# td-kwj-zp2023/webgpu-msm-twisted-edwards

Hardware: AMD Instinct MI355X
Metric: MSMs/sec at n=2^20 Twisted-Edwards BLS12 (pipelined throughput = 1000/ms_per_step; single-MSM latency in latency_ms) (higher is better)
Workload: dtype u32

## Files before the change

### webgpu-msm-twisted-edwards_amd/csrc/kernels.hip.hpp

```cpp
#pragma once
#include <hip/hip_runtime.h>
#include "curve.hpp"

namespace te {

#define TE_BATCH_MAX 8
struct batch_ptrs { const uint4* p[TE_BATCH_MAX]; };
struct batch_slabs { uint32_t s[TE_BATCH_MAX]; };

struct digits_params {
  uint32_t half[10];
  uint32_t zero_digit;
  uint32_t sc_stride;
  uint32_t n, nst;
  int num_windows;
  int w_first, w_step, nw_local;
  uint32_t half_code, logS, P, CH, chunk_len;
};

struct pnt_slot { uint4 q[8]; };
__device__ __forceinline__ void prep_points_block(uint32_t blk, uint4* __restrict__ lds, const uint4* __restrict__ pts, pnt_slot* __restrict__ recs, uint32_t n) {
  const uint32_t t = threadIdx.x, base = blk * 256u;
  const bool active = t < 256u;
  const uint32_t pieces_in = (n - base < 256u ? n - base : 256u) * 4u;
// ... 355 lines not shown
    prep_points_block(blk, lds4, in.p[row], recs + (size_t)row_slab.s[row] * n, n);
  }
}


struct piece_regs { uint4 k[5], ia[5], ib[5]; };
template <bool PK>
__device__ __forceinline__ void load_piece(const uint16_t* __restrict__ keys_row, const uint32_t* __restrict__ idx_row, uint32_t a, uint32_t b,
                                           uint32_t t, bool with_idx, piece_regs& r, uint32_t& head, uint32_t& total) {
  const uint32_t a_al = a & ~7u;
  head = a - a_al; total = head + (b - a);
  const uint32_t groups = (total + 7u) >> 3;
  const uint4* k4 = reinterpret_cast<const uint4*>(keys_row + a_al);
  const uint4* i4 = reinterpret_cast<const uint4*>(idx_row + a_al);
#pragma unroll
  for (int c = 0; c < 5; c++) {
    const uint32_t gi = min((uint32_t)c * 256u + t, groups - 1u);
    if (!PK) r.k[c] = k4[gi];
    if (PK || with_idx) { r.ia[c] = i4[2 * gi]; r.ib[c] = i4[2 * gi + 1]; }
  }
}
template <bool PK> __device__ __forceinline__ void piece_group(const piece_regs& r, int c, uint32_t (&kv)[8], uint32_t (&iv)[8]) {
  const uint32_t w[8] = {r.ia[c].x, r.ia[c].y, r.ia[c].z, r.ia[c].w, r.ib[c].x, r.ib[c].y, r.ib[c].z, r.ib[c].w};
  if (PK) {
#pragma unroll
    for (int e = 0; e < 8; e++) { kv[e] = ((w[e] >> 23) & 0xffu) | ((w[e] >> 31) << 15); iv[e] = w[e] & 0x7fffffu; }
  } else {
    unpack8(r.k[c], kv);
#pragma unroll
    for (int e = 0; e < 8; e++) iv[e] = w[e];
  }
}
static_assert(5u * 256u * 8u >= TE_L2_CAP + 8u, "five groups per thread hold a piece");

__device__ __forceinline__ bool l2_piece_of_block(uint32_t bx, const uint32_t* __restrict__ pc, uint32_t P, uint32_t overflow_pieces, uint32_t* sm, uint32_t* pj, uint32_t& p, uint32_t& j) {
  if (bx < P) { p = bx; j = 0u; return true; }
  const uint32_t t = threadIdx.x, x = bx - P;
  if (x >= overflow_pieces) return false;
  const uint32_t c = t < P ? pc[t] : 0u;
  const uint32_t ov = c ? (c + TE_L2_CAP - 1u) / TE_L2_CAP - 1u : 0u;
  uint32_t tot;
  const uint32_t ex = block_excl_scan(ov, sm, tot);
  if (x >= tot) return false;
  if (x >= ex && x < ex + ov) { pj[0] = t; pj[1] = x - ex + 1u; }
  __syncthreads();
  p = pj[0]; j = pj[1];
  __syncthreads();
  return true;
}

#define TE_COMBINE_SMALL 16u
#define TE_GIANT_RUN 256u
#define TE_SEG_INVALID 0xffffffffu
#define TE_HIST_COPIES 32u
struct plan_args {
  const uint32_t* part_start; const uint32_t* part_count; const uint32_t* seg_part_base;
  uint32_t *bucket_start, *bucket_cursor, *seg_base, *seg_bucket, *seg_lenv, *size_hist, *split_list;
  uint32_t* split_count;
  uint32_t* chunk_list;
  uint32_t seg_len, cap_w, chunk_cap;
};
struct plan_lds { uint32_t h[1024]; uint32_t sm[17]; uint32_t giant[256 * 3]; uint32_t n_giant; };
__device__ __forceinline__ uint32_t seg_plan_block(uint32_t p, uint32_t k, uint32_t cnt_in, const sort_geom& sg, const plan_args& a, plan_lds& L,
                                                   uint32_t pstart, uint32_t pcount, uint32_t sbase) {
  const uint32_t t = threadIdx.x, P = sg.P, S = sg.S, B = sg.B, seg_len = a.seg_len;
  uint32_t* const h = L.h; uint32_t* const sm = L.sm; uint32_t* const giant = L.giant;
  __syncthreads();
  for (uint32_t j = t; j < 1024u; j += 256u) h[j] = 0u;
  if (t == 0) L.n_giant = 0u;
  const bool mine = t < S;
  const uint32_t g = k * B + p * S + (mine ? t : 0u);
  const uint32_t cnt = mine ? cnt_in : 0u;
  const uint32_t nparts = mine ? max(1u, (cnt + seg_len - 1u) / seg_len) : 0u;
  uint32_t bt, bt2;
  const uint32_t ex = block_excl_scan(cnt, sm, bt);
  const uint32_t ex2 = block_excl_scan(nparts, sm, bt2);
  const uint32_t bs = pstart + ex, sb = sbase + ex2;
  if (mine) {
    a.bucket_start[g] = bs; a.bucket_cursor[g] = bs; a.seg_base[g] = sb;
    if (nparts <= TE_COMBINE_SMALL) {
      for (uint32_t part = 0; part < nparts; part++) {
        const uint32_t len = cnt > part * seg_len ? min(seg_len, cnt - part * seg_len) : 0u;
        a.seg_bucket[sb + part] = g; a.seg_lenv[sb + part] = len;
        atomicAdd(&h[min(len, 1023u)], 1u);
      }
      if (nparts > 1u) a.split_list[atomicAdd(&a.split_count[0], 1u)] = g;
    } else {
      const uint32_t j = atomicAdd(&L.n_giant, 1u);
      giant[3 * j] = g; giant[3 * j + 1] = sb; giant[3 * j + 2] = cnt;
      atomicAdd(&a.split_count[1], 1u);
    }
  }
  {
    const uint32_t first = sbase, used = bt2;
    const uint32_t cap = p + 1u == P ? (k + 1u) * a.cap_w - first : S + pcount / seg_len;
    for (uint32_t j = used + t; j < cap; j += 256u) { a.seg_bucket[first + j] = TE_SEG_INVALID; a.seg_lenv[first + j] = TE_SEG_INVALID; }
  }
  __syncthreads();
  const uint32_t ng = L.n_giant;
  for (uint32_t j = 0; j < ng; j++) {
    const uint32_t gg = giant[3 * j], sb0 = giant[3 * j + 1], c0 = giant[3 * j + 2];
    const uint32_t np = (c0 + seg_len - 1u) / seg_len;
    for (uint32_t part = t; part < np; part += 256u) {
      const uint32_t len = min(seg_len, c0 - part * seg_len);
      a.seg_bucket[sb0 + part] = gg; a.seg_lenv[sb0 + part] = len;
      atomicAdd(&h[min(len, 1023u)], 1u);
      if ((part & (TE_GIANT_RUN - 1u)) == 0) { const uint32_t ci = atomicAdd(&a.split_count[2], 1u); if (ci < a.chunk_cap) { a.chunk_list[2 * ci] = gg; a.chunk_list[2 * ci + 1] = part; } }
    }
  }
  __syncthreads();
  uint32_t* my_hist = a.size_hist + ((k * P + p) % TE_HIST_COPIES) * 1024u;
  for (uint32_t j = t; j < 1024u; j += 256u) if (h[j]) atomicAdd(&my_hist[j], h[j]);
  __syncthreads();
  return ex;
}

struct l2_args {
  const uint16_t* part_keys; const uint32_t* part_idx; const uint32_t* part_start; const uint32_t* part_count;
  uint32_t* bucket_count; uint32_t* sorted;
  uint32_t* part_ticket;
  sort_geom g; plan_args pa;
};
#define TE_L2A_LDS_WORDS (3u * 256u + 32u + TE_L2_LIST)
static_assert(sizeof(plan_lds) <= TE_L2_LIST * 4u, "the plan's LDS fits into the list area");
template <bool PK>
__global__ void __launch_bounds__(256, TE_L2_WAVES) k_l2_local(l2_args a) {
  __shared__ uint32_t lds[TE_L2A_LDS_WORDS];
  uint32_t* const cnt_s = lds; uint32_t* const off_s = lds + 256; uint32_t* const sm = lds + 768; uint32_t* const pj = lds + 768 + 17;
  uint32_t* const list = lds + 768 + 32;
  plan_lds& PL = *reinterpret_cast<plan_lds*>(list);
  const sort_geom& g = a.g;
  const uint32_t k = gridDim.y - 1u - blockIdx.y, t = threadIdx.x;
  const uint32_t extra = gridDim.x - g.P, bx = blockIdx.x < extra ? g.P + blockIdx.x : blockIdx.x - extra;
  const uint32_t* ps = a.part_start + k * g.P; const uint32_t* pc = a.part_count + k * g.P;
  uint32_t p, j;
  if (!l2_piece_of_block(bx, pc, g.P, bx < g.P ? 0u : a.part_count[gridDim.y * g.P + k], sm, pj, p, j)) return;
  const uint32_t cntp = pc[p], pb = ps[p], sbp = a.pa.seg_part_base[k * g.P + p];
  if (cntp == 0u) { (void)seg_plan_block(p, k, 0u, g, a.pa, PL, pb, cntp, sbp); return; }
  const bool single = cntp <= TE_L2_CAP;
  const uint32_t a0 = pb + j * TE_L2_CAP, b0 = min(pb + cntp, a0 + TE_L2_CAP);
  const uint16_t* keys_row = a.part_keys + (size_t)k * g.nst; const uint32_t* idx_row = a.part_idx + (size_t)k * g.nst;
  piece_regs r; uint32_t head, total;
  load_piece<PK>(keys_row, idx_row, a0, b0, t, single, r, head, total);
  cnt_s[t] = 0u;
  __syncthreads();
#pragma unroll
  for (int c = 0; c < 5; c++) {
    uint32_t kv[8], iv[8]; piece_group<PK>(r, c, kv, iv);
    const uint32_t e0 = ((uint32_t)c * 256u + t) * 8u;
#pragma unroll
    for (int e = 0; e < 8; e++) { const uint32_t pos = e0 + (uint32_t)e; if (pos >= head && pos < total) atomicAdd(&cnt_s[kv[e] & 0x7fffu], 1u); }
  }
  __syncthreads();
  const uint32_t c0 = cnt_s[t];
  const size_t gb = (size_t)k * g.B + (size_t)p * g.S + t;
  if (!single) {
    if (c0) atomicAdd(&a.bucket_count[gb], c0);
    wait_own_accesses();
// ... 198 lines not shown
  uint32_t w[4 * N];
#pragma unroll
  for (int j = 0; j < N; j++) { w[j] = a.x.v[j]; w[N + j] = a.y.v[j]; w[2 * N + j] = a.z.v[j]; w[3 * N + j] = a.t.v[j]; }
  uint4* o = reinterpret_cast<uint4*>(dst);
#pragma unroll
  for (int j = 0; j < N; j++) o[j] = make_uint4(w[4 * j], w[4 * j + 1], w[4 * j + 2], w[4 * j + 3]);
}
template <int N> __device__ __forceinline__ ete_t<N> load_ete(const ete_t<N>* src) {
  const uint4* q = reinterpret_cast<const uint4*>(src);
  uint32_t w[4 * N];
#pragma unroll
  for (int j = 0; j < N; j++) { const uint4 u = q[j]; w[4 * j] = u.x; w[4 * j + 1] = u.y; w[4 * j + 2] = u.z; w[4 * j + 3] = u.w; }
  ete_t<N> a;
#pragma unroll
  for (int j = 0; j < N; j++) { a.x.v[j] = w[j]; a.y.v[j] = w[N + j]; a.z.v[j] = w[2 * N + j]; a.t.v[j] = w[3 * N + j]; }
  return a;
}

struct __attribute__((aligned(8))) rec_aff377 { uint32_t w[42]; };
struct __attribute__((aligned(8))) u4a8 { uint32_t v[4]; };
struct __attribute__((aligned(8))) u2a8 { uint32_t v[2]; };
static_assert(sizeof(rec_aff377) == 168, "affine record slot");
__device__ __forceinline__ pnt_aff377 load_pnt_aff377(const rec_aff377* __restrict__ recs, uint32_t entry) {
  const uint32_t* base = recs[entry & 0x7fffffffu].w;
  u4a8 u[10];
#pragma unroll
  for (int j = 0; j < 10; j++) u[j] = reinterpret_cast<const u4a8*>(base)[j];
  const u2a8 t = *reinterpret_cast<const u2a8*>(base + 40);
  uint32_t w[42];
#pragma unroll
  for (int j = 0; j < 10; j++) { w[4 * j] = u[j].v[0]; w[4 * j + 1] = u[j].v[1]; w[4 * j + 2] = u[j].v[2]; w[4 * j + 3] = u[j].v[3]; }
  w[40] = t.v[0]; w[41] = t.v[1];
  pnt_aff377 r;
#pragma unroll
  for (int j = 0; j < 14; j++) { r.hm.v[j] = w[j]; r.hp.v[j] = w[14 + j]; r.dt.v[j] = w[28 + j]; }
  return r;
}
__device__ __forceinline__ void store_pnt_aff377(rec_aff377* dst, const pnt_aff377& r) {
#pragma unroll
  for (int j = 0; j < 14; j++) { dst->w[j] = r.hm.v[j]; dst->w[14 + j] = r.hp.v[j]; dst->w[28 + j] = r.dt.v[j]; }
}
template <int N, int RK> struct rec_kind;
template <int N> struct rec_kind<N, 0> {
  using slot = rec_slot<N>; using pnt = pnt_t<N>;
  static __device__ __forceinline__ pnt load(const slot* __restrict__ recs, uint32_t e) { return load_pnt<N>(recs, e); }
};
template <> struct rec_kind<14, 1> {
  using slot = rec_aff377; using pnt = pnt_aff377;
  static __device__ __forceinline__ pnt load(const slot* __restrict__ recs, uint32_t e) { return load_pnt_aff377(recs, e); }
};

struct __attribute__((aligned(4))) idx4 { uint32_t v[4]; };
#define TE_CLK_SLOTS 64u
#define TE_IDX_STRIP 16u
template <int N, int RK = 0>
__global__ void __launch_bounds__(256, N == 9 ? 3 : 2) k_accumulate(const typename rec_kind<N, RK>::slot* __restrict__ recs, const uint32_t* __restrict__ sorted,
                                                    const uint32_t* __restrict__ bucket_start, const uint32_t* __restrict__ bucket_count,
                                                    const uint32_t* __restrict__ seg_base, const uint32_t* __restrict__ seg_bucket,
                                                    const uint32_t* __restrict__ seg_lenv, const uint32_t* __restrict__ order,
                                                    const uint32_t* __restrict__ num_segments, ete_t<N>* __restrict__ buckets,
                                                    ete_t<N>* __restrict__ seg_out, uint32_t n, uint32_t logB, uint32_t seg_len, uint32_t ids, uint32_t onto,
                                                    uint32_t win_per_msm, batch_slabs slabs, unsigned long long* __restrict__ clk) {
  __shared__ uint32_t idx_strip[256 * TE_IDX_STRIP];
  using RT = rec_kind<N, RK>; using P = typename RT::pnt;
#if defined(TE_ACC_TWO_WAVES)
  if constexpr (N == 9) asm volatile("" ::: "v175");
#endif
  unsigned long long* const slot = clk ? clk + (blockIdx.x & (TE_CLK_SLOTS - 1u)) : nullptr;
  const unsigned long long t0_wall = clk ? (unsigned long long)wall_clock64() : 0ull, t0_core = clk ? (unsigned long long)clock64() : 0ull;
  if (clk && threadIdx.x == 0) atomicMax(slot, ~t0_wall);
  const uint32_t gid = blockIdx.x * 256u + threadIdx.x;
  if (gid >= (order ? *num_segments : ids)) return;
  const uint32_t sgm = order ? order[gid] : gid;
  const uint32_t g = seg_bucket[sgm];
  if (g == TE_SEG_INVALID) return;
  const uint32_t k = g >> logB;
  recs += (size_t)slabs.s[k / win_per_msm] * n;
  const uint32_t part = sgm - seg_base[g];
  const uint32_t cnt = seg_lenv[sgm];
  const uint32_t* lst = sorted + (size_t)k * n + bucket_start[g] + part * seg_len;
  ete_t<N> acc = (onto && part == 0u) ? load_ete<N>(buckets + g) : ete_identity_t<N>();
  if (cnt) {
    const uint32_t last = cnt - 1u;
    uint32_t j0 = 0;
    uint32_t e = lst[0], e_n = lst[min(1u, last)];
    P cur = RT::load(recs, e);
    if (!(onto && part == 0u)) {
      const P first = pnt_cneg(cur, (e >> 31) != 0u);
      e = e_n; e_n = lst[min(2u, last)];
      cur = RT::load(recs, e);
      acc = ete_from_pnt(first);
      j0 = 1;
    }
    uint32_t* const strip = idx_strip + threadIdx.x * TE_IDX_STRIP;
    auto refill = [&](uint32_t pos) {
      const idx4* src = reinterpret_cast<const idx4*>(lst + pos);
      idx4* dst = reinterpret_cast<idx4*>(strip);
#pragma unroll
      for (uint32_t h = 0; h < TE_IDX_STRIP / 4u; h += 2u) {
        const idx4 v0 = src[h], v1 = src[h + 1u];
        dst[h] = v0; dst[h + 1u] = v1;
      }
    };
    if (((j0 + 2u) & (TE_IDX_STRIP - 1u)) != 0u) refill((j0 + 2u) & ~(TE_IDX_STRIP - 1u));
    for (uint32_t j = j0; j < cnt; j++) {
      const uint32_t e_cur = e;
      P nxt = cur;
      const uint32_t pn = j + 2u;
      if ((pn & (TE_IDX_STRIP - 1u)) == 0u) refill(pn);
      const uint32_t e_nn = strip[pn & (TE_IDX_STRIP - 1u)];
      if (j + 1 < cnt) { e = e_n; nxt = RT::load(recs, e); }
      acc = ete_madd(acc, pnt_cneg(cur, (e_cur >> 31) != 0u));
      cur = nxt; e_n = e_nn;
    }
  }
  const bool whole = bucket_count[g] <= seg_len;
  store_ete<N>(whole ? buckets + g : seg_out + sgm, acc);
  if (clk && (uint32_t)__lane_id() == (uint32_t)__ffsll((long long)__ballot(1)) - 1u) {
    const unsigned long long t1_wall = (unsigned long long)wall_clock64(), t1_core = (unsigned long long)clock64();
    atomicMax(slot + TE_CLK_SLOTS, t1_wall);
    atomicAdd(slot + 2u * TE_CLK_SLOTS, t1_core - t0_core); atomicAdd(slot + 3u * TE_CLK_SLOTS, t1_wall - t0_wall);
  }
}

template <int N> struct sum_job_t {
  const ete_t<N>* in; ete_t<N>* out;
  uint32_t n_out;
  uint32_t K, inner;
  uint32_t in_per_window, out_per_window;
};
template <int N> struct sum_jobs_t { sum_job_t<N> j[4]; };
template <int N> __device__ __forceinline__ ete_t<N> pair_swap(const ete_t<N>& a) {
  ete_t<N> r;
#pragma unroll
  for (int i = 0; i < N; i++) {
    r.x.v[i] = (uint32_t)__builtin_amdgcn_mov_dpp((int)a.x.v[i], 0xb1, 0xf, 0xf, true);
    r.y.v[i] = (uint32_t)__builtin_amdgcn_mov_dpp((int)a.y.v[i], 0xb1, 0xf, 0xf, true);
    r.z.v[i] = (uint32_t)__builtin_amdgcn_mov_dpp((int)a.z.v[i], 0xb1, 0xf, 0xf, true);
    r.t.v[i] = (uint32_t)__builtin_amdgcn_mov_dpp((int)a.t.v[i], 0xb1, 0xf, 0xf, true);
  }
  return r;
}
template <int N, bool PAIR>
__global__ void __launch_bounds__(256, N == 9 ? 2 : 1) k_sum_groups(sum_jobs_t<N> js, uint32_t nw) {
  const sum_job_t<N>& j = js.j[blockIdx.y];
  constexpr uint32_t TPO = PAIR ? 2u : 1u;
  const uint32_t total = j.n_out * nw * TPO, Kt = j.K / TPO;
  for (uint32_t gt = blockIdx.x * 256u + threadIdx.x; gt < total; gt += gridDim.x * 256u) {
    const uint32_t g = gt / TPO, half = gt % TPO;
    const uint32_t k = g / j.n_out, o = g - k * j.n_out;
    const uint32_t outer = o / j.inner, q = o - outer * j.inner;
    const ete_t<N>* src = j.in + (size_t)k * j.in_per_window + ((size_t)outer * j.K + (size_t)half * Kt) * j.inner + q;
    ete_t<N> acc = load_ete<N>(src);
    if (Kt > 1u) {
      ete_t<N> nxt = load_ete<N>(src + (size_t)j.inner);
      for (uint32_t t = 1; t < Kt; t++) {
        const ete_t<N> cur = nxt;
        if (t + 1 < Kt) nxt = load_ete<N>(src + (size_t)(t + 1) * j.inner);
        acc = ete_add<N>(acc, cur);
      }
    }
    if (PAIR) {
      const ete_t<N> other = pair_swap<N>(acc);
      acc = ete_add<N>(acc, other);
      if (half != 0u) continue;
    }
    store_ete<N>(j.out + (size_t)k * j.out_per_window + o, acc);
  }
}
// ... 492 lines not shown
```

### webgpu-msm-twisted-edwards_amd/csrc/te_msm.hip

```cpp
#include <hip/hip_runtime.h>
#include <stdint.h>
#include <stdio.h>
#include <stdlib.h>
#include <string.h>
#include <string>
#include <vector>
#include <deque>
#include <algorithm>
#include <functional>
#include <chrono>
#include <thread>
#include <mutex>
#include <condition_variable>
#include <memory>
#if defined(__x86_64__)
#include <immintrin.h>
#endif

#include "../../include/te_msm.h"
#include "host_tail.hpp"
#include "synth.hpp"
#include "kernels.hip.hpp"
#include "check.hip.hpp"
#include "from_x.hip.hpp"
#include "scalar_mul.hip.hpp"
#include "probe.hip.hpp"
#include "host_tail377.hpp"
#include "host_sched.hpp"
#include "batch_plan.hpp"

namespace {

thread_local std::string g_init_error;

enum { ST_DIGITS = 0, ST_SCATTER, ST_BSORT, ST_ORDER, ST_PREP, ST_ACCUM, ST_TREE, ST_WEIGHTED, ST_COUNT };
const char* const kStageNames[ST_COUNT + 2] = {"digits", "part_scatter", "bucket_sort", "order", "prep_points",
                                               "accumulate", "marginal_sums", "weighted_sum", "accumulate_on_device", "accumulate_core_clock_ghz"};

struct curve_sizes { size_t point_in, scalar_in, acc, rec, row, result; };
inline curve_sizes sizes_of(int curve) {
  return curve == TE_MSM_CURVE_BLS12_377_G1 ? curve_sizes{96, 48, sizeof(te::ete_t<14>), sizeof(te::rec_slot<14>), TE377_TAIL_ROW_BYTES, 96}
                                            : curve_sizes{TE_MSM_POINT_BYTES, TE_MSM_SCALAR_BYTES, sizeof(te::ete), sizeof(te::rec_slot<9>), TE_MSM_PARTIAL_BYTES, 64};
}
inline size_t rec_bytes_of(int curve, int rec_kind) { return (curve == TE_MSM_CURVE_BLS12_377_G1 && rec_kind == 1) ? sizeof(te::rec_aff377) : sizes_of(curve).rec; }
static_assert(TE377_TAIL_ROW_BYTES == TE_MSM_PARTIAL_BYTES_BLS12_377 && sizeof(te::ete_t<14>) * 5 == TE377_TAIL_ROW_BYTES, "row layout");
constexpr size_t TE_MAX_ROW_BYTES = TE377_TAIL_ROW_BYTES;

struct plan_t {
  int curve = 0;
  int c = 0, W = 0, nw = 0;
  int nw1 = 0, batch = 1;
  int w_first = 0, w_step = 1;
  uint32_t B = 0, logB = 0;
  int signed_digits = 1;
  uint32_t dw[4] = {0, 0, 0, 0};
  uint32_t CH = 0, chunk_len = 0, nst = 0;
  uint32_t seg_len = 64;
  uint32_t S = 0, logS = 0, P = 0;
  uint32_t packed = 0;
  int rec_kind = 0;
  int fb_rb = 0, fb_c = 0, fb_W = 0;
};

struct graph_key { const void *pts, *sc, *out; uint64_t n, generation; int c, w_first, w_step, seg_len, sort; };

struct workset_t {
  hipStream_t stream = nullptr, copy_stream = nullptr;
  int hw_queue_class = -1;
  hipEvent_t ev_copy = nullptr, ev_start = nullptr;
  size_t cap[40] = {};
  uint8_t* d_recs = nullptr;
  uint16_t *d_digits = nullptr, *d_part_keys = nullptr;
  uint32_t *d_counts1 = nullptr, *d_part_start = nullptr, *d_part_count = nullptr, *d_part_idx = nullptr, *d_seg_part_base = nullptr;
  uint32_t *d_bucket_count = nullptr, *d_bucket_start = nullptr, *d_bucket_cursor = nullptr, *d_sorted = nullptr;
  uint32_t *d_seg_base = nullptr, *d_seg_bucket = nullptr, *d_seg_lenv = nullptr, *d_order = nullptr;
  uint32_t *d_split_list = nullptr, *d_chunk_list = nullptr;
  uint8_t *d_seg_out = nullptr, *d_buckets = nullptr, *d_red[4] = {};
  uint32_t *d_zero = nullptr; size_t zero_words = 0;
  size_t zero_clean_words = 0;
  uint32_t *d_err = nullptr, *d_num_seg = nullptr, *d_size_hist = nullptr, *d_size_cursor = nullptr;
  uint32_t* d_part_ticket = nullptr;
  uint8_t* d_partials = nullptr;
  uint32_t* h_err = nullptr;
  uint8_t* h_partials = nullptr;
  uint32_t* h_err_dev = nullptr;
  bool rows_on_host = false;
  hipEvent_t ev_done = nullptr;
  hipEvent_t ev_result = nullptr;
  hipEvent_t ev[ST_COUNT + 1] = {};
  plan_t plan; uint64_t n = 0; bool used = false;
  te_sched::slot_t slot;
  std::string job_err;
  int prof_level = 0;
  hipStream_t last_stream = nullptr;
  uint64_t generation = 0;
  hipGraphExec_t g_front = nullptr, g_back = nullptr; graph_key g_key = {};
  void *d_in_points = nullptr, *d_in_scalars = nullptr; size_t cap_in_points = 0, cap_in_scalars = 0;
  std::vector<hipEvent_t> piece_events;
  uint8_t* h_ring = nullptr; std::vector<hipEvent_t> ring_ev; size_t ring_next = 0;
  uint64_t idle_calls = 0;
  uint32_t* d_fb_remap = nullptr;
  uint32_t* d_fb_fill = nullptr;
  const void* fb_scalars = nullptr; uint64_t fb_n = 0;
  int slab = -1;
  bool slab_run = false;
  const uint8_t* recs_last = nullptr;
  te_bases* bound = nullptr;
  int pt_rc = 0; int64_t pt_index = -1; int pt_reason = 0;
  uint8_t* d_batch_rows = nullptr;
};
constexpr int TE_MAX_WINDOWS = 64;
constexpr size_t Z_KEEP = 4;
constexpr size_t Z_ENTRIES = 2;
constexpr size_t Z_CLOCK = 8;
static_assert(Z_KEEP + 4 <= Z_CLOCK && Z_ENTRIES % 2 == 0 && Z_ENTRIES + 2 <= Z_KEEP, "flag words");
constexpr size_t Z_ROWS = Z_CLOCK + 4 * 2 * TE_CLK_SLOTS, Z_HIST = Z_ROWS + (size_t)TE_MAX_WINDOWS * TE_MAX_ROW_BYTES / 4, Z_CURSOR = Z_HIST + 1024 * TE_HIST_COPIES, Z_END = Z_CURSOR + 1024;

struct gpu_t {
  int device = 0;
  int w_first = 0, w_step = 1;
  workset_t ws[TE_MSM_WORKSETS];
  int last_ws = 0;
  int wall_clock_khz = 0;
  int in_flight = 0;
  bool queues_probed = false;
  struct rec_slab_t { const void* src = nullptr; uint64_t n = 0; int curve = 0; uint8_t* d = nullptr; size_t cap = 0; int users = 0;
                      uint32_t pending = 0; hipEvent_t ev[TE_MSM_WORKSETS] = {};
                      int run_users = 0; bool converted = false; hipEvent_t conv_ev = nullptr; };
// ... 136 lines not shown
  p.chunk_len = (uint32_t)((p.nst + ch - 1) / ch);
  p.chunk_len = (p.chunk_len + 4095u) & ~4095u;
  ch = (p.nst + p.chunk_len - 1) / p.chunk_len;
  p.CH = ch;
  p.S = p.B < 256u ? p.B : 256u;
  if (force_seg) {
    p.seg_len = force_seg;
  } else if (ctx->opt_seg_len) {
    p.seg_len = (uint32_t)ctx->opt_seg_len;
  } else {
    uint64_t a = (2 * n + p.B - 1) / p.B, s2 = 16;
    while (s2 < a && s2 < 64) s2 <<= 1;
    p.seg_len = (uint32_t)s2;
  }
  p.P = p.B / p.S; p.logS = ilog2(p.S);
  p.packed = (ctx->opt_packed && n <= (1ull << 23)) ? 1u : 0u;
}

template <typename T> int ensure(te_ctx* ctx, workset_t& ws, T*& ptr, size_t& cap_bytes, size_t need_elems) {
  const size_t need = need_elems * sizeof(T);
  if (ptr && need <= cap_bytes) return 0;
  ws.generation++;
  if (ptr) HIP_TRY(ctx, hipFree(ptr));
  ptr = nullptr; cap_bytes = 0;
  HIP_TRY(ctx, hipMalloc((void**)&ptr, need ? need : 16));
  cap_bytes = need;
  return 0;
}

int ensure_buffers(te_ctx* ctx, gpu_t& d, workset_t& ws, uint64_t n, const plan_t& p, bool need_recs = true) {
  HIP_TRY(ctx, hipSetDevice(d.device));
  const size_t nd = (size_t)p.nw * p.nst + 64, wb = (size_t)p.nw * p.B, ab = sizes_of(p.curve).acc;
  int rc = 0;
  if (need_recs && (rc = ensure(ctx, ws, ws.d_recs, ws.cap[0], (size_t)n * sizes_of(p.curve).rec * (size_t)p.batch))) return rc;
  if ((rc = ensure(ctx, ws, ws.d_digits, ws.cap[1], nd))) return rc;
  if ((rc = ensure(ctx, ws, ws.d_sorted, ws.cap[2], nd))) return rc;
  {
    const size_t c1 = (size_t)p.nw * p.CH * p.P;
    ws.zero_words = Z_END + c1 + wb + (size_t)p.nw * p.P + 64;
    { const uint32_t* before = ws.d_zero; if ((rc = ensure(ctx, ws, ws.d_zero, ws.cap[3], ws.zero_words))) return rc; if (ws.d_zero != before) ws.zero_clean_words = 0; }
    ws.d_err = ws.d_zero; ws.d_num_seg = ws.d_zero + Z_KEEP; ws.d_size_hist = ws.d_zero + Z_HIST; ws.d_size_cursor = ws.d_zero + Z_CURSOR;
    ws.d_partials = reinterpret_cast<uint8_t*>(ws.d_zero + Z_ROWS);
    ws.d_counts1 = ws.d_zero + Z_END; ws.d_bucket_count = ws.d_counts1 + c1; ws.d_part_ticket = ws.d_bucket_count + wb;
    ws.d_fb_fill = ws.d_part_ticket + (size_t)p.nw * p.P;
  }
  if (p.fb_rb && (rc = ensure(ctx, ws, ws.d_fb_remap, ws.cap[27], nd))) return rc;
  if ((rc = ensure(ctx, ws, ws.d_bucket_start, ws.cap[5], wb))) return rc;
  if ((rc = ensure(ctx, ws, ws.d_bucket_cursor, ws.cap[16], wb))) return rc;
  if ((rc = ensure(ctx, ws, ws.d_seg_part_base, ws.cap[17], (size_t)p.nw * p.P))) return rc;
  const size_t smax = wb + (size_t)p.nw * (n / (uint64_t)p.seg_len) + 16;
  if ((rc = ensure(ctx, ws, ws.d_order, ws.cap[7], smax))) return rc;
  if ((rc = ensure(ctx, ws, ws.d_seg_bucket, ws.cap[20], smax))) return rc;
  if ((rc = ensure(ctx, ws, ws.d_seg_lenv, ws.cap[21], smax))) return rc;
  if ((rc = ensure(ctx, ws, ws.d_seg_out, ws.cap[22], smax * ab))) return rc;
  if ((rc = ensure(ctx, ws, ws.d_seg_base, ws.cap[23], wb + 1))) return rc;
  if ((rc = ensure(ctx, ws, ws.d_split_list, ws.cap[24], wb + 1))) return rc;
  if ((rc = ensure(ctx, ws, ws.d_chunk_list, ws.cap[26], 2 * (wb + smax / TE_GIANT_RUN + 2)))) return rc;
  if ((rc = ensure(ctx, ws, ws.d_part_start, ws.cap[6], (size_t)p.nw * p.P))) return rc;
  if ((rc = ensure(ctx, ws, ws.d_buckets, ws.cap[8], wb * ab))) return rc;
  if ((rc = ensure(ctx, ws, ws.d_part_count, ws.cap[9], (size_t)p.nw * p.P + (size_t)p.nw))) return rc;
  if ((rc = ensure(ctx, ws, ws.d_part_keys, ws.cap[14], p.packed ? 8 : nd))) return rc;
  if ((rc = ensure(ctx, ws, ws.d_part_idx, ws.cap[15], nd))) return rc;
  if ((rc = ensure(ctx, ws, ws.d_red[0], ws.cap[10], (wb / 2 + 1) * ab))) return rc;
  if ((rc = ensure(ctx, ws, ws.d_red[1], ws.cap[11], (wb / 4 + 1) * ab))) return rc;
  if ((rc = ensure(ctx, ws, ws.d_red[2], ws.cap[12], (wb / 2 + 1) * ab))) return rc;
  if ((rc = ensure(ctx, ws, ws.d_red[3], ws.cap[13], (wb / 4 + 1) * ab))) return rc;
  return 0;
}

template <int C> void launch_digits(const te::batch_ptrs& sc, int batch, uint16_t* dg, const te::digits_params& prm, uint32_t* err, uint32_t* counts1, hipStream_t s) {
  hipLaunchKernelGGL(te::k_digits<C>, dim3((prm.nst + TE_DIG_BLOCK - 1u) / TE_DIG_BLOCK, batch), dim3(TE_DIG_THREADS), 0, s, sc, dg, prm, err, counts1);
}
static_assert(TE_BATCH_MAX == TE_MSM_MAX_BATCH, "batch tables");
template <int C> void launch_digits_ragged(const void* sc, const te::ragged_tab& tab, int batch, uint16_t* dg, const te::digits_params& prm, uint32_t* err, uint32_t* counts1, hipStream_t s) {
  hipLaunchKernelGGL(te::k_digits_ragged<C>, dim3((prm.nst + TE_DIG_BLOCK - 1u) / TE_DIG_BLOCK, batch), dim3(TE_DIG_THREADS), 0, s, static_cast<const uint4*>(sc), tab, dg, prm, err, counts1);
}
static_assert(TE_RAGGED_MAX == TE_BATCH_SEQ_MAX && TE_BATCH_SEQ_MAX == TE_MSM_BATCH_SEQ_MAX, "ragged tables");

struct msm_launch {
  te_ctx* ctx; gpu_t& d; workset_t& ws; plan_t p;
  const void* d_points; const void* d_scalars; uint64_t n; void* d_partials_out;
  int prof;
  hipStream_t stream;
  bool own_rows = false;
  bool onto = false;
  bool host_rows = false;
  uint8_t* recs_rw = nullptr;
  uint8_t* recs_out() const { return recs_rw ? recs_rw : ws.d_recs; }
  bool have_recs = false;
  void count_conversion() const { __atomic_fetch_add(&ctx->stat_record_conversions, (int64_t)1, __ATOMIC_RELAXED); }
  const uint32_t* fb_remap = nullptr;
  int table_replicas = 1;
  const uint8_t* bound = nullptr;
  const te::ragged_tab* ragged = nullptr;
  static bool rows_to_host(const te_ctx* ctx, const gpu_t& d, const plan_t& p, bool own_rows) {
    return own_rows && p.nw > 0 && p.batch == 1 && p.w_first == 0 && p.w_step == 1 && ctx->opt_prezero && !ctx->opt_graph;
  }
  uint32_t n32() const { return (uint32_t)n; }
  uint32_t total() const { return (uint32_t)p.nw * p.B; }
  uint32_t smax() const { return total() + (uint32_t)((uint64_t)p.nw * (n / p.seg_len)); }
  uint32_t chunk_cap() const { return total() + smax() / TE_GIANT_RUN + 2u; }
  const void* points_of(int m) const { return p.batch > 1 ? static_cast<const void* const*>(d_points)[m] : d_points; }
  const void* scalars_of(int m) const { return p.batch > 1 ? static_cast<const void* const*>(d_scalars)[m] : d_scalars; }
  void mark(int i) const { if (prof >= 2 || (prof == 1 && (i == ST_ACCUM || i == ST_ACCUM + 1))) (void)hipEventRecord(ws.ev[i], stream); }

  bool can_fuse_prep() const { return ctx->opt_fuse_prep && prof < 2 && p.nw > 0; }
// ... 69 lines not shown
          case 12: launch_digits_ragged<12>(d_scalars, *ragged, p.batch, dg, prm, ws.d_err, c1, stream); break;
          case 13: launch_digits_ragged<13>(d_scalars, *ragged, p.batch, dg, prm, ws.d_err, c1, stream); break;
          case 14: launch_digits_ragged<14>(d_scalars, *ragged, p.batch, dg, prm, ws.d_err, c1, stream); break;
          case 15: launch_digits_ragged<15>(d_scalars, *ragged, p.batch, dg, prm, ws.d_err, c1, stream); break;
          default: launch_digits_ragged<16>(d_scalars, *ragged, p.batch, dg, prm, ws.d_err, c1, stream); break;
        }
      } else switch (p.c) {
        case 4: launch_digits<4>(sc, p.batch, dg, prm, ws.d_err, c1, stream); break;
        case 5: launch_digits<5>(sc, p.batch, dg, prm, ws.d_err, c1, stream); break;
        case 6: launch_digits<6>(sc, p.batch, dg, prm, ws.d_err, c1, stream); break;
        case 7: launch_digits<7>(sc, p.batch, dg, prm, ws.d_err, c1, stream); break;
        case 8: launch_digits<8>(sc, p.batch, dg, prm, ws.d_err, c1, stream); break;
        case 9: launch_digits<9>(sc, p.batch, dg, prm, ws.d_err, c1, stream); break;
        case 10: launch_digits<10>(sc, p.batch, dg, prm, ws.d_err, c1, stream); break;
        case 11: launch_digits<11>(sc, p.batch, dg, prm, ws.d_err, c1, stream); break;
        case 12: launch_digits<12>(sc, p.batch, dg, prm, ws.d_err, c1, stream); break;
        case 13: launch_digits<13>(sc, p.batch, dg, prm, ws.d_err, c1, stream); break;
        case 14: launch_digits<14>(sc, p.batch, dg, prm, ws.d_err, c1, stream); break;
        case 15: launch_digits<15>(sc, p.batch, dg, prm, ws.d_err, c1, stream); break;
        default: launch_digits<16>(sc, p.batch, dg, prm, ws.d_err, c1, stream); break;
      }
    }
    const uint32_t cap_w = p.B + (uint32_t)(n / p.seg_len);
    mark(ST_SCATTER);
    if (p.nw > 0) {
      te::scatter_args sa;
      sa.digits = ws.d_digits; sa.counts1 = ws.d_counts1; sa.part_keys = ws.d_part_keys; sa.part_idx = ws.d_part_idx; sa.part_start = ws.d_part_start;
      sa.part_count = ws.d_part_count; sa.seg_part_base = ws.d_seg_part_base; sa.entries = reinterpret_cast<unsigned long long*>(ws.d_zero + Z_ENTRIES); sa.seg_len = p.seg_len; sa.cap_w = cap_w; sa.nw = (uint32_t)p.nw; sa.g = sg; sa.remap = fb_remap; sa.row_fill = ws.d_fb_fill;
      if (with_prep) {
        te::batch_ptrs tab; te::batch_slabs row_slab;
        const uint32_t rows = (uint32_t)prep_rows(tab, row_slab), sblocks = p.CH * (uint32_t)p.nw;
        count_conversion();
        if (bls()) {
          const uint32_t per_row = (n32 + 511u) / 512u;
          hipLaunchKernelGGL(te::k_part_scatter_prep377, dim3(sblocks + rows * per_row), dim3(512), 0, stream, sa, sblocks, tab, row_slab,
                             reinterpret_cast<te::rec_slot<14>*>(recs_out()), n32, per_row, rows * per_row);
        } else {
          const uint32_t per_row = (n32 + 255u) / 256u;
          hipLaunchKernelGGL(te::k_part_scatter_prep, dim3(sblocks + rows * per_row), dim3(512), 0, stream, sa, sblocks, tab, row_slab,
                             reinterpret_cast<te::pnt_slot*>(recs_out()), n32, per_row, rows * per_row);
        }
      } else {
        hipLaunchKernelGGL(te::k_part_scatter, dim3(p.CH, p.nw), dim3(512), 0, stream, sa);
      }
    }
    mark(ST_BSORT);
    if (p.nw > 0) {
      const uint32_t l2_blocks = p.P + n32 / TE_L2_CAP + 1u;
      te::l2_args la;
      la.part_keys = ws.d_part_keys; la.part_idx = ws.d_part_idx; la.part_start = ws.d_part_start; la.part_count = ws.d_part_count;
      la.bucket_count = ws.d_bucket_count; la.sorted = ws.d_sorted; la.part_ticket = ws.d_part_ticket; la.g = sg;
      la.pa.part_start = ws.d_part_start; la.pa.part_count = ws.d_part_count; la.pa.seg_part_base = ws.d_seg_part_base;
      la.pa.bucket_start = ws.d_bucket_start; la.pa.bucket_cursor = ws.d_bucket_cursor; la.pa.seg_base = ws.d_seg_base; la.pa.seg_bucket = ws.d_seg_bucket;
      la.pa.seg_lenv = ws.d_seg_lenv; la.pa.size_hist = ws.d_size_hist; la.pa.split_list = ws.d_split_list; la.pa.split_count = ws.d_num_seg + 1;
      la.pa.chunk_list = ws.d_chunk_list; la.pa.seg_len = p.seg_len; la.pa.cap_w = cap_w; la.pa.chunk_cap = chunk_cap();
      if (p.packed) hipLaunchKernelGGL(te::k_l2_local<true>, dim3(l2_blocks, p.nw), dim3(256), 0, stream, la);
      else hipLaunchKernelGGL(te::k_l2_local<false>, dim3(l2_blocks, p.nw), dim3(256), 0, stream, la);
      te::order_args oa;
      oa.lenv = ws.d_seg_lenv; oa.ids = smax(); oa.size_hist = ws.d_size_hist; oa.rel_cursor = ws.d_size_cursor; oa.order = ws.d_order; oa.num_segments = ws.d_num_seg;
      {
        const uint32_t by_regs = (smax() + TE_ORDER_REGS * 256u * (uint32_t)p.nw - 1u) / (TE_ORDER_REGS * 256u * (uint32_t)p.nw);
        oa.order_cols = std::min(64u, std::max(by_regs, (uint32_t)std::max(1, 128 / p.nw)));
      }
      oa.max_len = std::min(p.seg_len, 1023u);
      if (p.packed)
        hipLaunchKernelGGL(te::k_l2_place_order<true>, dim3(oa.order_cols + l2_blocks, p.nw), dim3(256), 0, stream, ws.d_part_keys, ws.d_part_idx, ws.d_part_start,
                           ws.d_part_count, ws.d_bucket_cursor, ws.d_sorted, sg, oa);
      else
        hipLaunchKernelGGL(te::k_l2_place_order<false>, dim3(oa.order_cols + l2_blocks, p.nw), dim3(256), 0, stream, ws.d_part_keys, ws.d_part_idx, ws.d_part_start,
                           ws.d_part_count, ws.d_bucket_cursor, ws.d_sorted, sg, oa);
    }
    mark(ST_ORDER);
    return 0;
  }

  bool bls() const { return p.curve == TE_MSM_CURVE_BLS12_377_G1; }

  template <int N, int RK> int accumulate_t() {
    mark(ST_ACCUM);
    if (p.nw > 0) {
      const uint32_t n32 = this->n32(), smax = this->smax();
      const uint32_t* order = ctx->opt_sort ? ws.d_order : nullptr;
      using slot_t = typename te::rec_kind<N, RK>::slot;
      static const bool serial = [] { const char* e = getenv("TE_MSM_SERIAL_ACCUMULATE"); return e && e[0] == '1'; }();
      std::unique_lock<std::mutex> chain(*d.acc_mu, std::defer_lock);
      if (serial && !ctx->opt_graph) {
        chain.lock();
        if (d.acc_prev && d.acc_prev_stream != stream) HIP_TRY(ctx, hipStreamWaitEvent(stream, d.acc_prev, 0));
      }
      hipLaunchKernelGGL((te::k_accumulate<N, RK>), dim3((smax + 255) / 256), dim3(256), 0, stream, reinterpret_cast<const slot_t*>(bound ? bound : recs_out()), ws.d_sorted,
                         ws.d_bucket_start, ws.d_bucket_count, ws.d_seg_base, ws.d_seg_bucket, ws.d_seg_lenv, order, ws.d_num_seg,
                         reinterpret_cast<te::ete_t<N>*>(ws.d_buckets), reinterpret_cast<te::ete_t<N>*>(ws.d_seg_out), n32, p.logB, p.seg_len, smax, onto ? 1u : 0u,
                         ragged ? (uint32_t)p.nw : table_replicas > 1 ? (uint32_t)((p.nw1 + table_replicas - 1) / table_replicas) : (uint32_t)p.nw1,
                         ragged ? te::batch_slabs{} : table_replicas > 1 ? replica_slabs() : slabs(),
                         prof ? reinterpret_cast<unsigned long long*>(ws.d_zero + Z_CLOCK) : nullptr);
      if (chain.owns_lock()) {
        hipEvent_t& ev = d.acc_ev[d.acc_next++ % 16u];
        if (!ev) HIP_TRY(ctx, hipEventCreateWithFlags(&ev, hipEventDisableTiming));
        HIP_TRY(ctx, hipEventRecord(ev, stream));
        d.acc_prev = ev; d.acc_prev_stream = stream;
      }
    }
    return 0;
  }
  int accumulate() { return bls() ? (p.rec_kind == 1 ? accumulate_t<14, 1>() : accumulate_t<14, 0>()) : accumulate_t<9, 0>(); }

  template <int N> int combine_t() {
    if (p.nw <= 0) return 0;
    using E = te::ete_t<N>;
    hipLaunchKernelGGL(te::k_seg_combine_all<N>, dim3(256 + 1024), dim3(256), 0, stream, ws.d_split_list, ws.d_num_seg + 1, ws.d_chunk_list,
                       ws.d_bucket_count, ws.d_seg_base, reinterpret_cast<E*>(ws.d_seg_out), reinterpret_cast<E*>(ws.d_buckets), p.seg_len, chunk_cap(), 256u,
                       ws.d_bucket_start, ws.d_bucket_cursor);
    return 0;
  }
  int combine() { return bls() ? combine_t<14>() : combine_t<9>(); }

  template <int N> int reduce_t() {
    if (p.nw > 0) {
      using E = te::ete_t<N>;
      const uint32_t w0 = p.dw[0], w1 = p.dw[1], w2 = p.dw[2], w3 = p.dw[3];
      const uint32_t L = 1u << (w0 + w1), H = 1u << (w2 + w3);
      struct chain_t { const E* cur; uint32_t n, r; E* buf[2]; int pp; };
      E* const bk = reinterpret_cast<E*>(ws.d_buckets);
      chain_t ch[2] = {{bk, p.B, L, {reinterpret_cast<E*>(ws.d_red[0]), reinterpret_cast<E*>(ws.d_red[1])}, 0},
                       {bk, p.B, H, {reinterpret_cast<E*>(ws.d_red[2]), reinterpret_cast<E*>(ws.d_red[3])}, 0}};
      for (;;) {
        te::sum_jobs_t<N> js; memset(&js, 0, sizeof js);
        uint32_t most = 0; int nj = 0;
        for (int i = 0; i < 2; i++) {
          chain_t& c = ch[i];
          if (c.r <= 4u) continue;
          const uint32_t K = (c.r % 8u == 0) ? 8u : (c.r % 4u == 0) ? 4u : 2u;
          te::sum_job_t<N>& j = js.j[nj++];
          j.in = c.cur; j.out = c.buf[c.pp]; j.K = K; j.n_out = c.n / K;
          j.inner = i == 0 ? c.r / K : (c.r / K) * L;
          j.in_per_window = c.n; j.out_per_window = c.n / K;
          c.cur = j.out; c.pp ^= 1; c.r /= K; c.n /= K;
          most = std::max(most, j.n_out * (uint32_t)p.nw);
        }
        if (!nj) break;
        if (most >= 65536u || (most >= 32768u && !ctx->opt_fold_pairs)) {
          uint32_t blocks = (most + 255) / 256; if (blocks > 4096) blocks = 4096;
          hipLaunchKernelGGL((te::k_sum_groups<N, false>), dim3(blocks, nj), dim3(256), 0, stream, js, (uint32_t)p.nw);
        } else if (most >= 32768u) {
          uint32_t blocks = (2 * most + 255) / 256; if (blocks > 4096) blocks = 4096;
// ... 307 lines not shown
    if (int rc = L.back()) return rc;
  }
  if (!own_rows) { if (int rc = finish_sequence(ctx, ws, stream)) return rc; }
  HIP_TRY(ctx, hipGetLastError());
  guard.armed = false;
  return 0;
}

int fetch_rows(te_ctx* ctx, workset_t& ws, hipStream_t stream) {
  if (!ws.rows_on_host)
    HIP_TRY(ctx, hipMemcpyAsync(ws.h_err, ws.d_zero, Z_ROWS * 4 + (size_t)ws.plan.W * sizes_of(ws.plan.curve).row, hipMemcpyDeviceToHost, stream));
  return finish_sequence(ctx, ws, stream);
}

int finish_sequence(te_ctx* ctx, workset_t& ws, hipStream_t stream) {
  HIP_TRY(ctx, hipEventRecord(ws.ev_result, stream));
  if (ctx->opt_prezero && !ctx->opt_graph) {
    HIP_TRY(ctx, hipMemsetAsync(ws.d_zero, 0, ws.zero_words * sizeof(uint32_t), stream));
    ws.zero_clean_words = ws.zero_words;
  }
  HIP_TRY(ctx, hipEventRecord(ws.ev_done, stream));
  return 0;
}

int collect_stage_ms(te_ctx* ctx, const gpu_t& d, workset_t& ws) {
  if (!ws.prof_level) return 0;
  bool ok = true;
  for (int i = 0; i < ST_COUNT; i++) {
    float ms = -1.0f;
    if (ws.prof_level >= 2 || i == ST_ACCUM) ok = ok && hipEventElapsedTime(&ms, ws.ev[i], ws.ev[i + 1]) == hipSuccess;
    ctx->stage_ms[i] = ms;
  }
  {
    uint64_t raw[4 * TE_CLK_SLOTS]; memcpy(raw, ws.h_err + Z_CLOCK, sizeof raw);
    uint64_t c[4] = {0, 0, 0, 0};
    for (uint32_t i = 0; i < TE_CLK_SLOTS; i++) {
      c[0] = std::max(c[0], raw[i]); c[1] = std::max(c[1], raw[TE_CLK_SLOTS + i]);
      c[2] += raw[2 * TE_CLK_SLOTS + i]; c[3] += raw[3 * TE_CLK_SLOTS + i];
    }
    const int khz = d.wall_clock_khz;
    const bool have = c[0] && c[1] && khz > 0 && c[1] > ~c[0];
    const double ms = have ? (double)(c[1] - ~c[0]) / khz : -1.0;
    ctx->stage_ms[ST_COUNT] = (float)ms;
    ctx->stage_ms[ST_COUNT + 1] = (have && c[2] && c[3]) ? (float)((double)c[2] / (double)c[3] * khz * 1e-6) : -1.0f;
  }
  if (!ok) (void)hipGetLastError();
  ctx->have_stage_ms = ok;
  return 0;
}

void free_workset_buffers(workset_t& ws) {
  void** ptrs[] = {(void**)&ws.d_recs, (void**)&ws.d_digits, (void**)&ws.d_part_keys, (void**)&ws.d_zero, (void**)&ws.d_part_start, (void**)&ws.d_part_count,
                   (void**)&ws.d_part_idx, (void**)&ws.d_seg_part_base, (void**)&ws.d_bucket_start, (void**)&ws.d_bucket_cursor, (void**)&ws.d_sorted,
                   (void**)&ws.d_seg_base, (void**)&ws.d_seg_bucket, (void**)&ws.d_seg_lenv, (void**)&ws.d_order, (void**)&ws.d_split_list,
                   (void**)&ws.d_chunk_list, (void**)&ws.d_seg_out, (void**)&ws.d_buckets, (void**)&ws.d_red[0], (void**)&ws.d_red[1],
                   (void**)&ws.d_red[2], (void**)&ws.d_red[3], &ws.d_in_points, &ws.d_in_scalars, (void**)&ws.d_fb_remap, (void**)&ws.d_batch_rows};
  for (void** q : ptrs) if (*q) { (void)hipFree(*q); *q = nullptr; }
  if (ws.h_ring) { (void)hipHostFree(ws.h_ring); ws.h_ring = nullptr; }
  memset(ws.cap, 0, sizeof ws.cap); ws.cap_in_points = ws.cap_in_scalars = 0;
  ws.zero_words = ws.zero_clean_words = 0;
  ws.d_err = ws.d_num_seg = ws.d_size_hist = ws.d_size_cursor = ws.d_counts1 = ws.d_bucket_count = ws.d_part_ticket = nullptr; ws.d_partials = nullptr;
  if (ws.g_front) { (void)hipGraphExecDestroy(ws.g_front); ws.g_front = nullptr; }
  if (ws.g_back) { (void)hipGraphExecDestroy(ws.g_back); ws.g_back = nullptr; }
  ws.generation++; ws.used = false;
}

void free_dev(gpu_t& d) {
  (void)hipSetDevice(d.device);
  for (auto& sl : d.slabs) {
    if (sl.d) { (void)hipFree(sl.d); sl.d = nullptr; }
    for (hipEvent_t& e : sl.ev) if (e) { (void)hipEventDestroy(e); e = nullptr; }
    if (sl.conv_ev) { (void)hipEventDestroy(sl.conv_ev); sl.conv_ev = nullptr; }
  }
  d.slabs.clear();
  for (hipEvent_t& e : d.acc_ev) { if (e) (void)hipEventDestroy(e); e = nullptr; }
  d.acc_prev = nullptr; d.acc_prev_stream = nullptr;
  if (d.chk_stream) (void)hipStreamDestroy(d.chk_stream);
  if (d.chk_pts) (void)hipFree(d.chk_pts);
  if (d.chk_word) (void)hipFree(d.chk_word);
  if (d.chk_host) (void)hipHostFree(d.chk_host);
  d.chk_stream = nullptr; d.chk_pts = nullptr; d.chk_cap = 0; d.chk_word = d.chk_host = nullptr;
  if (d.h_batch_rows) (void)hipHostFree(d.h_batch_rows);
  d.h_batch_rows = nullptr; d.h_batch_cap = 0;
  for (workset_t& ws : d.ws) {
    free_workset_buffers(ws);
    if (ws.h_err) (void)hipHostFree(ws.h_err);
    for (hipEvent_t e : ws.ring_ev) if (e) (void)hipEventDestroy(e);
    if (ws.ev_done) (void)hipEventDestroy(ws.ev_done);
    if (ws.ev_result) (void)hipEventDestroy(ws.ev_result);
    for (auto& ev : ws.ev) if (ev) (void)hipEventDestroy(ev);
    if (ws.ev_copy) (void)hipEventDestroy(ws.ev_copy);
    if (ws.ev_start) (void)hipEventDestroy(ws.ev_start);
    for (hipEvent_t e : ws.piece_events) (void)hipEventDestroy(e);
    if (ws.copy_stream) (void)hipStreamDestroy(ws.copy_stream);
    if (ws.stream) { if (d.streams_exported && park_exported_streams()) park_stream(d.device, ws.stream); else (void)hipStreamDestroy(ws.stream); }
    ws.stream = nullptr; ws.copy_stream = nullptr;
  }
}

int ensure_staging(te_ctx* ctx, workset_t& ws, size_t bytes_points, size_t bytes_scalars) {
  if (bytes_points > ws.cap_in_points) {
    if (ws.d_in_points) HIP_TRY(ctx, hipFree(ws.d_in_points));
    ws.d_in_points = nullptr; ws.cap_in_points = 0;
    HIP_TRY(ctx, hipMalloc(&ws.d_in_points, bytes_points));
    ws.cap_in_points = bytes_points;
  }
  if (bytes_scalars > ws.cap_in_scalars) {
// ... 2184 lines not shown
```

Measured before the change: 1123.

## Pack per-segment metadata into one uint4 record and widen index strip

The planning kernel now also writes a packed per-segment record holding the bucket id, the absolute start offset, and the length with first-part and whole-bucket flags. The accumulate kernel reads that single 16-byte record instead of making several dependent gathers (seg_bucket, seg_base, seg_lenv, bucket_start, bucket_count). This shortens its startup latency chain. The LDS index strip doubles to 32 entries with batched loads, and refills are now bounded by the segment length. The cost is extra global writes in the plan kernel, more shared memory per block (which may cut occupancy), and a new buffer.

```diff
diff --git a/webgpu-msm-twisted-edwards_amd/csrc/kernels.hip.hpp b/webgpu-msm-twisted-edwards_amd/csrc/kernels.hip.hpp
--- a/webgpu-msm-twisted-edwards_amd/csrc/kernels.hip.hpp
+++ b/webgpu-msm-twisted-edwards_amd/csrc/kernels.hip.hpp
@@ -431,15 +431,19 @@
 #define TE_COMBINE_SMALL 16u
 #define TE_GIANT_RUN 256u
 #define TE_SEG_INVALID 0xffffffffu
+#define TE_SEG_FIRST 0x40000000u
+#define TE_SEG_WHOLE 0x80000000u
+#define TE_SEG_LEN_MASK 0x3fffffffu
 #define TE_HIST_COPIES 32u
 struct plan_args {
   const uint32_t* part_start; const uint32_t* part_count; const uint32_t* seg_part_base;
   uint32_t *bucket_start, *bucket_cursor, *seg_base, *seg_bucket, *seg_lenv, *size_hist, *split_list;
+  uint4* seg_rec;
   uint32_t* split_count;
   uint32_t* chunk_list;
   uint32_t seg_len, cap_w, chunk_cap;
 };
-struct plan_lds { uint32_t h[1024]; uint32_t sm[17]; uint32_t giant[256 * 3]; uint32_t n_giant; };
+struct plan_lds { uint32_t h[1024]; uint32_t sm[17]; uint32_t giant[256 * 4]; uint32_t n_giant; };
 __device__ __forceinline__ uint32_t seg_plan_block(uint32_t p, uint32_t k, uint32_t cnt_in, const sort_geom& sg, const plan_args& a, plan_lds& L,
                                                    uint32_t pstart, uint32_t pcount, uint32_t sbase) {
   const uint32_t t = threadIdx.x, P = sg.P, S = sg.S, B = sg.B, seg_len = a.seg_len;
@@ -461,28 +465,32 @@
       for (uint32_t part = 0; part < nparts; part++) {
         const uint32_t len = cnt > part * seg_len ? min(seg_len, cnt - part * seg_len) : 0u;
         a.seg_bucket[sb + part] = g; a.seg_lenv[sb + part] = len;
+        a.seg_rec[sb + part] = make_uint4(g, bs + part * seg_len, len | (part == 0u ? TE_SEG_FIRST : 0u) | (nparts == 1u ? TE_SEG_WHOLE : 0u), 0u);
         atomicAdd(&h[min(len, 1023u)], 1u);
       }
       if (nparts > 1u) a.split_list[atomicAdd(&a.split_count[0], 1u)] = g;
     } else {
       const uint32_t j = atomicAdd(&L.n_giant, 1u);
-      giant[3 * j] = g; giant[3 * j + 1] = sb; giant[3 * j + 2] = cnt;
+      giant[4 * j] = g; giant[4 * j + 1] = sb; giant[4 * j + 2] = cnt; giant[4 * j + 3] = bs;
       atomicAdd(&a.split_count[1], 1u);
     }
   }
   {
     const uint32_t first = sbase, used = bt2;
     const uint32_t cap = p + 1u == P ? (k + 1u) * a.cap_w - first : S + pcount / seg_len;
-    for (uint32_t j = used + t; j < cap; j += 256u) { a.seg_bucket[first + j] = TE_SEG_INVALID; a.seg_lenv[first + j] = TE_SEG_INVALID; }
+    for (uint32_t j = used + t; j < cap; j += 256u) {
+      a.seg_bucket[first + j] = TE_SEG_INVALID; a.seg_lenv[first + j] = TE_SEG_INVALID; a.seg_rec[first + j] = make_uint4(TE_SEG_INVALID, 0u, 0u, 0u);
+    }
   }
   __syncthreads();
   const uint32_t ng = L.n_giant;
   for (uint32_t j = 0; j < ng; j++) {
-    const uint32_t gg = giant[3 * j], sb0 = giant[3 * j + 1], c0 = giant[3 * j + 2];
+    const uint32_t gg = giant[4 * j], sb0 = giant[4 * j + 1], c0 = giant[4 * j + 2], bs0 = giant[4 * j + 3];
     const uint32_t np = (c0 + seg_len - 1u) / seg_len;
     for (uint32_t part = t; part < np; part += 256u) {
       const uint32_t len = min(seg_len, c0 - part * seg_len);
       a.seg_bucket[sb0 + part] = gg; a.seg_lenv[sb0 + part] = len;
+      a.seg_rec[sb0 + part] = make_uint4(gg, bs0 + part * seg_len, len | (part == 0u ? TE_SEG_FIRST : 0u), 0u);
       atomicAdd(&h[min(len, 1023u)], 1u);
       if ((part & (TE_GIANT_RUN - 1u)) == 0) { const uint32_t ci = atomicAdd(&a.split_count[2], 1u); if (ci < a.chunk_cap) { a.chunk_list[2 * ci] = gg; a.chunk_list[2 * ci + 1] = part; } }
     }
@@ -787,14 +795,12 @@
 
 struct __attribute__((aligned(4))) idx4 { uint32_t v[4]; };
 #define TE_CLK_SLOTS 64u
-#define TE_IDX_STRIP 16u
+#define TE_IDX_STRIP 32u
 template <int N, int RK = 0>
 __global__ void __launch_bounds__(256, N == 9 ? 3 : 2) k_accumulate(const typename rec_kind<N, RK>::slot* __restrict__ recs, const uint32_t* __restrict__ sorted,
-                                                    const uint32_t* __restrict__ bucket_start, const uint32_t* __restrict__ bucket_count,
-                                                    const uint32_t* __restrict__ seg_base, const uint32_t* __restrict__ seg_bucket,
-                                                    const uint32_t* __restrict__ seg_lenv, const uint32_t* __restrict__ order,
+                                                    const uint4* __restrict__ seg_rec, const uint32_t* __restrict__ order,
                                                     const uint32_t* __restrict__ num_segments, ete_t<N>* __restrict__ buckets,
-                                                    ete_t<N>* __restrict__ seg_out, uint32_t n, uint32_t logB, uint32_t seg_len, uint32_t ids, uint32_t onto,
+                                                    ete_t<N>* __restrict__ seg_out, uint32_t n, uint32_t logB, uint32_t ids, uint32_t onto,
                                                     uint32_t win_per_msm, batch_slabs slabs, unsigned long long* __restrict__ clk) {
   __shared__ uint32_t idx_strip[256 * TE_IDX_STRIP];
   using RT = rec_kind<N, RK>; using P = typename RT::pnt;
@@ -807,20 +813,21 @@
   const uint32_t gid = blockIdx.x * 256u + threadIdx.x;
   if (gid >= (order ? *num_segments : ids)) return;
   const uint32_t sgm = order ? order[gid] : gid;
-  const uint32_t g = seg_bucket[sgm];
+  const uint4 sr = seg_rec[sgm];
+  const uint32_t g = sr.x;
   if (g == TE_SEG_INVALID) return;
   const uint32_t k = g >> logB;
   recs += (size_t)slabs.s[k / win_per_msm] * n;
-  const uint32_t part = sgm - seg_base[g];
-  const uint32_t cnt = seg_lenv[sgm];
-  const uint32_t* lst = sorted + (size_t)k * n + bucket_start[g] + part * seg_len;
-  ete_t<N> acc = (onto && part == 0u) ? load_ete<N>(buckets + g) : ete_identity_t<N>();
+  const bool first_part = (sr.z & TE_SEG_FIRST) != 0u;
+  const uint32_t cnt = sr.z & TE_SEG_LEN_MASK;
+  const uint32_t* lst = sorted + (size_t)k * n + sr.y;
+  ete_t<N> acc = (onto && first_part) ? load_ete<N>(buckets + g) : ete_identity_t<N>();
   if (cnt) {
     const uint32_t last = cnt - 1u;
     uint32_t j0 = 0;
     uint32_t e = lst[0], e_n = lst[min(1u, last)];
     P cur = RT::load(recs, e);
-    if (!(onto && part == 0u)) {
+    if (!(onto && first_part)) {
       const P first = pnt_cneg(cur, (e >> 31) != 0u);
       e = e_n; e_n = lst[min(2u, last)];
       cur = RT::load(recs, e);
@@ -831,25 +838,25 @@
     auto refill = [&](uint32_t pos) {
       const idx4* src = reinterpret_cast<const idx4*>(lst + pos);
       idx4* dst = reinterpret_cast<idx4*>(strip);
-#pragma unroll
-      for (uint32_t h = 0; h < TE_IDX_STRIP / 4u; h += 2u) {
-        const idx4 v0 = src[h], v1 = src[h + 1u];
-        dst[h] = v0; dst[h + 1u] = v1;
-      }
+      idx4 v[TE_IDX_STRIP / 4u];
+#pragma unroll
+      for (uint32_t h = 0; h < TE_IDX_STRIP / 4u; h++) v[h] = src[h];
+#pragma unroll
+      for (uint32_t h = 0; h < TE_IDX_STRIP / 4u; h++) dst[h] = v[h];
     };
-    if (((j0 + 2u) & (TE_IDX_STRIP - 1u)) != 0u) refill((j0 + 2u) & ~(TE_IDX_STRIP - 1u));
+    if (j0 + 2u < cnt) refill(0u);
     for (uint32_t j = j0; j < cnt; j++) {
       const uint32_t e_cur = e;
       P nxt = cur;
       const uint32_t pn = j + 2u;
-      if ((pn & (TE_IDX_STRIP - 1u)) == 0u) refill(pn);
+      if ((pn & (TE_IDX_STRIP - 1u)) == 0u && pn < cnt) refill(pn);
       const uint32_t e_nn = strip[pn & (TE_IDX_STRIP - 1u)];
       if (j + 1 < cnt) { e = e_n; nxt = RT::load(recs, e); }
       acc = ete_madd(acc, pnt_cneg(cur, (e_cur >> 31) != 0u));
       cur = nxt; e_n = e_nn;
     }
   }
-  const bool whole = bucket_count[g] <= seg_len;
+  const bool whole = (sr.z & TE_SEG_WHOLE) != 0u;
   store_ete<N>(whole ? buckets + g : seg_out + sgm, acc);
   if (clk && (uint32_t)__lane_id() == (uint32_t)__ffsll((long long)__ballot(1)) - 1u) {
     const unsigned long long t1_wall = (unsigned long long)wall_clock64(), t1_core = (unsigned long long)clock64();
diff --git a/webgpu-msm-twisted-edwards_amd/csrc/te_msm.hip b/webgpu-msm-twisted-edwards_amd/csrc/te_msm.hip
--- a/webgpu-msm-twisted-edwards_amd/csrc/te_msm.hip
+++ b/webgpu-msm-twisted-edwards_amd/csrc/te_msm.hip
@@ -74,6 +74,7 @@
   uint32_t *d_counts1 = nullptr, *d_part_start = nullptr, *d_part_count = nullptr, *d_part_idx = nullptr, *d_seg_part_base = nullptr;
   uint32_t *d_bucket_count = nullptr, *d_bucket_start = nullptr, *d_bucket_cursor = nullptr, *d_sorted = nullptr;
   uint32_t *d_seg_base = nullptr, *d_seg_bucket = nullptr, *d_seg_lenv = nullptr, *d_order = nullptr;
+  uint4* d_seg_rec = nullptr;
   uint32_t *d_split_list = nullptr, *d_chunk_list = nullptr;
   uint8_t *d_seg_out = nullptr, *d_buckets = nullptr, *d_red[4] = {};
   uint32_t *d_zero = nullptr; size_t zero_words = 0;
@@ -316,6 +317,7 @@
   if ((rc = ensure(ctx, ws, ws.d_order, ws.cap[7], smax))) return rc;
   if ((rc = ensure(ctx, ws, ws.d_seg_bucket, ws.cap[20], smax))) return rc;
   if ((rc = ensure(ctx, ws, ws.d_seg_lenv, ws.cap[21], smax))) return rc;
+  if ((rc = ensure(ctx, ws, ws.d_seg_rec, ws.cap[29], smax))) return rc;
   if ((rc = ensure(ctx, ws, ws.d_seg_out, ws.cap[22], smax * ab))) return rc;
   if ((rc = ensure(ctx, ws, ws.d_seg_base, ws.cap[23], wb + 1))) return rc;
   if ((rc = ensure(ctx, ws, ws.d_split_list, ws.cap[24], wb + 1))) return rc;
@@ -491,7 +493,7 @@
       la.bucket_count = ws.d_bucket_count; la.sorted = ws.d_sorted; la.part_ticket = ws.d_part_ticket; la.g = sg;
       la.pa.part_start = ws.d_part_start; la.pa.part_count = ws.d_part_count; la.pa.seg_part_base = ws.d_seg_part_base;
       la.pa.bucket_start = ws.d_bucket_start; la.pa.bucket_cursor = ws.d_bucket_cursor; la.pa.seg_base = ws.d_seg_base; la.pa.seg_bucket = ws.d_seg_bucket;
-      la.pa.seg_lenv = ws.d_seg_lenv; la.pa.size_hist = ws.d_size_hist; la.pa.split_list = ws.d_split_list; la.pa.split_count = ws.d_num_seg + 1;
+      la.pa.seg_lenv = ws.d_seg_lenv; la.pa.seg_rec = ws.d_seg_rec; la.pa.size_hist = ws.d_size_hist; la.pa.split_list = ws.d_split_list; la.pa.split_count = ws.d_num_seg + 1;
       la.pa.chunk_list = ws.d_chunk_list; la.pa.seg_len = p.seg_len; la.pa.cap_w = cap_w; la.pa.chunk_cap = chunk_cap();
       if (p.packed) hipLaunchKernelGGL(te::k_l2_local<true>, dim3(l2_blocks, p.nw), dim3(256), 0, stream, la);
       else hipLaunchKernelGGL(te::k_l2_local<false>, dim3(l2_blocks, p.nw), dim3(256), 0, stream, la);
@@ -528,8 +530,8 @@
         if (d.acc_prev && d.acc_prev_stream != stream) HIP_TRY(ctx, hipStreamWaitEvent(stream, d.acc_prev, 0));
       }
       hipLaunchKernelGGL((te::k_accumulate<N, RK>), dim3((smax + 255) / 256), dim3(256), 0, stream, reinterpret_cast<const slot_t*>(bound ? bound : recs_out()), ws.d_sorted,
-                         ws.d_bucket_start, ws.d_bucket_count, ws.d_seg_base, ws.d_seg_bucket, ws.d_seg_lenv, order, ws.d_num_seg,
-                         reinterpret_cast<te::ete_t<N>*>(ws.d_buckets), reinterpret_cast<te::ete_t<N>*>(ws.d_seg_out), n32, p.logB, p.seg_len, smax, onto ? 1u : 0u,
+                         ws.d_seg_rec, order, ws.d_num_seg,
+                         reinterpret_cast<te::ete_t<N>*>(ws.d_buckets), reinterpret_cast<te::ete_t<N>*>(ws.d_seg_out), n32, p.logB, smax, onto ? 1u : 0u,
                          ragged ? (uint32_t)p.nw : table_replicas > 1 ? (uint32_t)((p.nw1 + table_replicas - 1) / table_replicas) : (uint32_t)p.nw1,
                          ragged ? te::batch_slabs{} : table_replicas > 1 ? replica_slabs() : slabs(),
                          prof ? reinterpret_cast<unsigned long long*>(ws.d_zero + Z_CLOCK) : nullptr);
@@ -943,7 +945,7 @@
 void free_workset_buffers(workset_t& ws) {
   void** ptrs[] = {(void**)&ws.d_recs, (void**)&ws.d_digits, (void**)&ws.d_part_keys, (void**)&ws.d_zero, (void**)&ws.d_part_start, (void**)&ws.d_part_count,
                    (void**)&ws.d_part_idx, (void**)&ws.d_seg_part_base, (void**)&ws.d_bucket_start, (void**)&ws.d_bucket_cursor, (void**)&ws.d_sorted,
-                   (void**)&ws.d_seg_base, (void**)&ws.d_seg_bucket, (void**)&ws.d_seg_lenv, (void**)&ws.d_order, (void**)&ws.d_split_list,
+                   (void**)&ws.d_seg_base, (void**)&ws.d_seg_bucket, (void**)&ws.d_seg_lenv, (void**)&ws.d_seg_rec, (void**)&ws.d_order, (void**)&ws.d_split_list,
                    (void**)&ws.d_chunk_list, (void**)&ws.d_seg_out, (void**)&ws.d_buckets, (void**)&ws.d_red[0], (void**)&ws.d_red[1],
                    (void**)&ws.d_red[2], (void**)&ws.d_red[3], &ws.d_in_points, &ws.d_in_scalars, (void**)&ws.d_fb_remap, (void**)&ws.d_batch_rows};
   for (void** q : ptrs) if (*q) { (void)hipFree(*q); *q = nullptr; }
```

Result: no change. 1121 (median of 4 runs) (-0.1%).
